# ooowedyn/InkLayer

Hardware: AMD Instinct MI355X
Metric: sketches/sec end-to-end (GroundingDINO+SAM) at 1024x1024 (higher is better)
Workload: dtype f16 (MFMA, f32 accumulate; f32 residual/norm/softmax; split-f16 = fp32-grade operands for patch-embed, neck, mask decoder); 1 GPU; full GroundingDINO Swin-T + SAM ViT-H pipeline, batch=8 per GPU, 1024x1024 synthetic sketches, 16 boxes/sketch, random-init weights; global_batch=8, parallelism=image-parallel x1

## Files before the change

inklayer_amd/build.py:

```python
from __future__ import annotations

import os
import subprocess
import sys
from concurrent.futures import ThreadPoolExecutor
from pathlib import Path

ROOT = Path(__file__).resolve().parent
CSRC = ROOT / "csrc"
LIBDIR = ROOT / "lib"
OBJDIR = LIBDIR / "obj"
LIB = LIBDIR / "libinklayer_hip.so"
HIPCC = os.environ.get("HIPCC", "/opt/rocm/bin/hipcc")
FLAGS = ["--offload-arch=gfx950", "-O3", "-std=c++17", "-fPIC", "-ffp-contract=off",
         "-mllvm", "-amdgpu-mfma-vgpr-form",

         "-Wall", "-Wno-unused-function", "-Wno-unused-variable"]


def _newest_header() -> float:
    hs = list(CSRC.glob("*.h")) + list((ROOT.parent / "include").glob("*.h"))
    return max(h.stat().st_mtime for h in hs)


NO_SPILL = {"ffn_fused.hip", "proj_ln.hip", "amg.hip", "layers.hip", "inpaint_ops.hip", "visualize.hip", "evaluate.hip",
            "gemm.hip", "attention_swin.hip", "biattn_wide.hip", "text_bert.hip"}


def _check_no_spill(src: Path, remarks: str) -> None:
    name = None
    for line in remarks.splitlines():
        if "Function Name:" in line:
            name = line.split("Function Name:")[1].split("[")[0].strip()
        elif "ScratchSize [bytes/lane]:" in line:
            n = int(line.split("ScratchSize [bytes/lane]:")[1].split("[")[0])
            if n != 0:
                raise RuntimeError(f"{src.name}: kernel {name} spills ({n} bytes of scratch per lane) - the kernels of "
                                   f"this file must stay in registers (see NO_SPILL); reduce register pressure")


def _compile(src: Path, force: bool, hdr_time: float) -> Path:
    obj = OBJDIR / (src.stem + ".o")
    if (not force and obj.exists() and obj.stat().st_mtime > src.stat().st_mtime
            and obj.stat().st_mtime > hdr_time):
        return obj
    guard = src.name in NO_SPILL
    cmd = [HIPCC, *FLAGS, *(["-Rpass-analysis=kernel-resource-usage", "-fno-caret-diagnostics"] if guard else []), "-c", str(src), "-o", str(obj)]
    r = subprocess.run(cmd, capture_output=True, text=True)
    if r.returncode != 0:
        raise RuntimeError(f"hipcc failed for {src.name}:\n{r.stdout}\n{r.stderr}")
    err = r.stderr
    if guard:
        try:
            _check_no_spill(src, err)
        except RuntimeError:
            obj.unlink(missing_ok=True)
            raise
        err = "\n".join(l for l in err.splitlines()
                        if "kernel-resource-usage" not in l and not l.startswith("In file included from"))
    if err.strip():
        sys.stderr.write(err)
    return obj


def build(force: bool = False, verbose: bool = True) -> Path:
    OBJDIR.mkdir(parents=True, exist_ok=True)
    srcs = sorted(CSRC.glob("*.hip"))
    if not srcs:
        raise RuntimeError("no HIP sources found")
    hdr_time = _newest_header()
    with ThreadPoolExecutor(max_workers=min(8, len(srcs))) as ex:
        objs = list(ex.map(lambda s: _compile(s, force, hdr_time), srcs))
    if (force or not LIB.exists()
            or any(o.stat().st_mtime > LIB.stat().st_mtime for o in objs)):
        cmd = [HIPCC, "--offload-arch=gfx950", "-shared", "-fPIC", "-o", str(LIB),
               *map(str, objs)]
        r = subprocess.run(cmd, capture_output=True, text=True)
        if r.returncode != 0:
            raise RuntimeError(f"link failed:\n{r.stdout}\n{r.stderr}")
    if verbose:
        print(f"[inklayer_amd.build] {LIB} ({LIB.stat().st_size >> 10} KiB, {len(srcs)} sources)")
    return LIB


if __name__ == "__main__":
    build(force="--force" in sys.argv)
```

inklayer_amd/csrc/attention_glob.hip:

```cpp
#include "mfma_util.h"
#include "../../include/inklayer_hip.h"

namespace {

typedef int i32x4 __attribute__((ext_vector_type(4)));

constexpr int HD = 80, NT = 256, NQK = 5, NB = 3, CH = 10;
constexpr int KROW = 176, VROW = 192;
constexpr int TILE = 64 * KROW + 64 * VROW;
constexpr int RWROW = 272;
constexpr int LDS_BYTES = 2 * TILE + 256 * RWROW;
constexpr int OROW = 176;
static_assert(4 * 64 * OROW <= 2 * TILE, "the output tiles fit the K/V buffers");
constexpr float NEG = -1e30f;
constexpr float THR = 12.0f;

struct Sub {
  f16x8 qf[NQK];
  f32x16 s0, s1;
  uint32_t pw[16];
  f32x16 o[NB];
  float m, nm;
  float mx, mx2, ea, eb, fa, fb;
  __device__ __forceinline__ f16x8 pfrag(int ks) const {
    typedef uint32_t u32x4 __attribute__((ext_vector_type(4)));
    return __builtin_bit_cast(f16x8, (u32x4){pw[4 * ks], pw[4 * ks + 1], pw[4 * ks + 2], pw[4 * ks + 3]});
  }
};

__device__ __forceinline__ void s_mfma(int j, const f16x8 (&kfa)[NQK], const f16x8 (&kfb)[NQK], Sub& u) {
  const int s = j >> 1;
  if (j & 1) u.s1 = mfma32(kfb[s], u.qf[s], u.s1);
  else u.s0 = mfma32(kfa[s], u.qf[s], u.s0);
}
__device__ __forceinline__ void pv_mfma(int j, const f16x8 (&vf)[12], Sub& u) {
  u.o[j % 3] = mfma32(vf[j], u.pfrag(j / 3), u.o[j % 3]);
}
__device__ __forceinline__ void sm_max(int g, Sub& u) {
  if (g == 0) {
    u.mx = max3_at(u.s0[0], u.s0[1], u.s0[2]);
    u.mx2 = max3_at(u.s0[3], u.s0[4], u.s0[5]);
    u.mx = max3_at(u.mx, u.s0[6], u.s0[7]);
    u.mx2 = max3_at(u.mx2, u.s0[8], u.s0[9]);
    u.mx = max3_at(u.mx, u.s0[10], u.s0[11]);
    u.mx2 = max3_at(u.mx2, u.s0[12], u.s0[13]);
  } else if (g == 1) {
    u.mx = max3_at(u.mx, u.s0[14], u.s0[15]);
    u.mx2 = max3_at(u.mx2, u.s1[0], u.s1[1]);
    u.mx = max3_at(u.mx, u.s1[2], u.s1[3]);
    u.mx2 = max3_at(u.mx2, u.s1[4], u.s1[5]);
    u.mx = max3_at(u.mx, u.s1[6], u.s1[7]);
  } else {
    u.mx2 = max3_at(u.mx2, u.s1[8], u.s1[9]);
    u.mx = max3_at(u.mx, u.s1[10], u.s1[11]);
    u.mx2 = max3_at(u.mx2, u.s1[12], u.s1[13]);
    u.mx = max3_at(u.mx, u.s1[14], u.s1[15]);
    u.mx = fmaxf(u.mx, u.mx2);
  }
}
template <bool FIRST>
__device__ __forceinline__ void sm_decide(Sub& u, float c, float rh) {
  float x = u.mx, y = u.mx;
  asm volatile("s_nop 1\n\tv_permlane32_swap_b32 %0, %1" : "+v"(x), "+v"(y));
  const float mc = (fmaxf(x, y) + rh) * c;
  if constexpr (FIRST) {
    u.m = mc;
  } else {
    if (__any(mc - u.m > THR)) {
      const float m_new = fmaxf(u.m, mc);
      const float alpha = __builtin_amdgcn_exp2f(u.m - m_new);
#pragma unroll
      for (int i = 0; i < NB; ++i)
#pragma unroll
        for (int r2 = 0; r2 < 16; ++r2) u.o[i][r2] *= alpha;
      u.m = m_new;
    }
  }
  u.nm = rh * c - u.m;
}
__device__ __forceinline__ void sm_exp(int i, Sub& u, float c) {
  float pa = 0.f, pb = 0.f;
  if (i >= 2 && i < 18) { pa = u.ea; pb = u.eb; }
  if (i >= 1 && i < 17) {
    u.ea = exp2_at(u.fa);
    u.eb = exp2_at(u.fb);
  }
  if (i < 16) {
    float a, b;
    if (i < 8) { a = u.s0[2 * i]; b = u.s0[2 * i + 1]; }
    else { a = u.s1[2 * i - 16]; b = u.s1[2 * i - 15]; }
    u.fa = fma_at(a, c, u.nm);
    u.fb = fma_at(b, c, u.nm);
  }
  if (i >= 2 && i < 18) u.pw[i - 2] = cvt_pk_at(pa, pb);
}
template <bool FIRST>
__device__ __forceinline__ void sm_first(int g, Sub& u, float c, float rh) {
  if (g < 3) sm_max(g, u);
  else if (g == 3) sm_decide<FIRST>(u, c, rh);
  else sm_exp(g - 4, u, c);
}
__device__ __forceinline__ void sm_second(int g, Sub& u, float c) { sm_exp(8 + g, u, c); }

template <bool RF16>
__global__ __launch_bounds__(NT) __attribute__((amdgpu_waves_per_eu(1, 1))) void glob4_attn_kernel(InkAttn p) {
  using RT = std::conditional_t<RF16, f16, float>;
  extern __shared__ __attribute__((aligned(16))) char smem[];
  asm volatile("v_accvgpr_write_b32 a255, %0" ::"v"(0) : "a255");
  char* sRW = smem + 2 * TILE;

  const int tid = threadIdx.x, lane = tid & 63;
  const int wave = __builtin_amdgcn_readfirstlane(tid >> 6);
  const int lq = lane & 31, hh = lane >> 5;
  const int nqb = p.n_q >> 8;
  const int blk = xcd_remap((int)blockIdx.x, (int)gridDim.x);
  const int bh = blk / nqb, qb = blk - bh * nqb;
  const int b = bh / p.n_heads, h = bh - b * p.n_heads;
  const int ntiles = p.n_k >> 6;
  const int64_t qrow0 = p.q_batch_rows ? (int64_t)p.q_batch_rows[b] : (int64_t)b * p.n_q;
  const int64_t kvb = p.kv_batch_rows ? (int64_t)p.kv_batch_rows[b] : (int64_t)b * p.n_k;
  const int qlA = wave * 32 + lq, qlB = 128 + wave * 32 + lq;

  Sub A, B;
  auto load_q = [&](Sub& u, int ql) {
    const int64_t q = (int64_t)qb * 256 + ql;
    const f16* Qrow = (const f16*)p.Q + (qrow0 + q) * p.ldq + h * HD + 8 * hh;
#pragma unroll
    for (int s = 0; s < NQK; ++s) u.qf[s] = *(const f16x8*)(Qrow + 16 * s);
  };
  load_q(A, qlA);
  load_q(B, qlB);
  {
    const RT* RW = (const RT*)p.rel_w + ((int64_t)bh * p.n_q + (int64_t)qb * 256) * 64;
#pragma unroll
    for (int it = 0; it < 16; ++it) {
      const int ci = it * NT + tid, q = ci >> 4, c4 = ci & 15;
      if constexpr (RF16) {
        const f16x4 v = *(const f16x4*)(RW + q * 64 + c4 * 4);
        *(f32x4*)(sRW + q * RWROW + c4 * 16) = (f32x4){(float)v[0], (float)v[1], (float)v[2], (float)v[3]};
      } else {
        *(f32x4*)(sRW + q * RWROW + c4 * 16) = *(const f32x4*)(RW + q * 64 + c4 * 4);
      }
    }
  }
  const RT* RHA = (const RT*)p.rel_h + ((int64_t)bh * p.n_q + (int64_t)qb * 256 + qlA) * 64;
  const RT* RHB = (const RT*)p.rel_h + ((int64_t)bh * p.n_q + (int64_t)qb * 256 + qlB) * 64;
  for (int i = tid; i < 2 * 64 * 2; i += NT) {
    const int buf = i >> 7, row = (i >> 1) & 63, pc = i & 1;
    f16x8 z = {0, 0, 0, 0, 0, 0, 0, 0};
    if (pc == 0) { z[0] = (f16)1; z[4] = (f16)1; }
    *(f16x8*)(smem + buf * TILE + 64 * KROW + row * VROW + (CH + pc) * 16) = z;
  }

  const char* Kg = (const char*)p.K + (kvb * p.ldk + h * HD) * 2;
  const char* Vg = (const char*)p.V + (kvb * p.ldv + h * HD) * 2;
  uint32_t goff[5];
  int loff[5];
  bool isv[5];
#pragma unroll
  for (int it = 0; it < 5; ++it) {
    const int ci = it * NT + tid;
    const bool v = ci >= 640;
    const int cj = v ? ci - 640 : ci, row = cj / CH, cc = cj - row * CH;
    isv[it] = v;
    goff[it] = (uint32_t)(row * (v ? p.ldv : p.ldk) * 2 + cc * 16);
    loff[it] = v ? 64 * KROW + row * VROW + cc * 16 : row * KROW + cc * 16;
  }
  f16x8 stg[2][5];
  const char* gp[5];
#pragma unroll
  for (int it = 0; it < 5; ++it) gp[it] = (isv[it] ? Vg : Kg) + goff[it];
  const int64_t kstride = (int64_t)64 * p.ldk * 2, vstride = (int64_t)64 * p.ldv * 2;
  auto g_load = [&](int tile, auto SET, auto IT) {
    constexpr int set = decltype(SET)::value, it = decltype(IT)::value;
    stg[set][it] = *(const f16x8*)gp[it];
    const int64_t step = tile + 1 < ntiles ? (isv[it] ? vstride : kstride) : 0;
    gp[it] += step;
  };
  auto l_write = [&](int buf, auto SET, auto IT) {
    constexpr int set = decltype(SET)::value, it = decltype(IT)::value;
    *(f16x8*)(smem + buf * TILE + loff[it]) = stg[set][it];
  };
  static_for<0, 5>([&](auto it) { g_load(0, ic<0>{}, it); });
  static_for<0, 5>([&](auto it) { g_load(1, ic<1>{}, it); });
  static_for<0, 5>([&](auto it) { l_write(0, ic<0>{}, it); });
  static_for<0, 5>([&](auto it) { l_write(1, ic<1>{}, it); });
  static_for<0, 5>([&](auto it) { g_load(2, ic<0>{}, it); });
  __syncthreads();

  const float c = p.scale * 1.44269504088896340736f;
  const int koff0 = lq * KROW + hh * 16;
  const int koff1 = (32 + lq) * KROW + hh * 16;
  const int voff = 64 * KROW + (4 * hh + ((lane & 15) >> 2)) * VROW + (16 * ((lane >> 4) & 1) + 4 * (lane & 3)) * 2;
#pragma unroll
  for (int i = 0; i < NB; ++i)
#pragma unroll
    for (int r = 0; r < 16; ++r) A.o[i][r] = B.o[i][r] = 0.f;
  A.m = B.m = NEG;
  A.nm = B.nm = 0.f;
  f16x8 kfa[NQK], kfb[NQK], vf[12];
  auto read_k = [&](int buf, int s) {
    kfa[s] = *(const f16x8*)(smem + buf * TILE + koff0 + s * 32);
    kfb[s] = *(const f16x8*)(smem + buf * TILE + koff1 + s * 32);
  };
  auto read_v = [&](int buf, int j) {
    const char* base = smem + buf * TILE + voff + (16 * (j / 3)) * VROW + (j % 3) * 64;
    const f16x4 a0 = tr_read(base);
    const f16x4 a1 = tr_read(base + 8 * VROW);
    vf[j] = (f16x8){a0[0], a0[1], a0[2], a0[3], a1[0], a1[1], a1[2], a1[3]};
  };
#define GAP() __builtin_amdgcn_sched_barrier(0)

  auto read_rw = [&](Sub& u, int ql, int g) {
    const f32x4 a = *(const f32x4*)(sRW + ql * RWROW + (8 * g + 4 * hh) * 4);
    const f32x4 c2 = *(const f32x4*)(sRW + ql * RWROW + (32 + 8 * g + 4 * hh) * 4);
#pragma unroll
    for (int r = 0; r < 4; ++r) { u.s0[4 * g + r] = a[r]; u.s1[4 * g + r] = c2[r]; }
  };
  float rhA = (float)RHA[0], rhB = (float)RHB[0];
#pragma unroll
  for (int g = 0; g < 4; ++g) { read_rw(A, qlA, g); read_rw(B, qlB, g); }
#pragma unroll
  for (int s = 0; s < NQK; ++s) read_k(0, s);
#pragma unroll
  for (int j = 0; j < 10; ++j) s_mfma(j, kfa, kfb, A);
  GAP();

  auto tile_iter = [&](int t, auto PAR_, auto FIRST_) {
    constexpr int PAR = decltype(PAR_)::value;
    constexpr bool FIRST = decltype(FIRST_)::value;
    float rhA1 = 0.f, rhB1 = 0.f;
    if constexpr (FIRST) {
      static_for<0, 10>([&](auto g_) {
        constexpr int g = decltype(g_)::value;
        s_mfma(g, kfa, kfb, B);
        sm_first<true>(g, A, c, rhA);
        read_v(PAR, g);
        if constexpr (g == 9) { read_v(PAR, 10); read_v(PAR, 11); }
        if constexpr (g % 4 == 1) g_load(t + 3, ic<1 - PAR>{}, ic<g / 4>{});
        GAP();
      });
      static_for<10, 12>([&](auto g_) { sm_first<true>(decltype(g_)::value, A, c, rhA); GAP(); });
      static_for<0, 10>([&](auto g_) {
        constexpr int g = decltype(g_)::value;
        sm_second(g, A, c);
        if constexpr (g == 2) g_load(t + 3, ic<1 - PAR>{}, ic<3>{});
        if constexpr (g == 6) g_load(t + 3, ic<1 - PAR>{}, ic<4>{});
        GAP();
      });
    } else {
      static_for<0, 12>([&](auto g_) {
        constexpr int g = decltype(g_)::value;
        pv_mfma(g, vf, B);
        sm_first<false>(g, A, c, rhA);
        if constexpr (g % 4 == 2) g_load(t + 3, ic<1 - PAR>{}, ic<g / 4>{});
        if constexpr (g >= 8) read_rw(B, qlB, g - 8);
        GAP();
      });
      static_for<0, 10>([&](auto g_) {
        constexpr int g = decltype(g_)::value;
        s_mfma(g, kfa, kfb, B);
        sm_second(g, A, c);
        read_v(PAR, g);
        if constexpr (g == 9) { read_v(PAR, 10); read_v(PAR, 11); }
        if constexpr (g == 3) g_load(t + 3, ic<1 - PAR>{}, ic<3>{});
        if constexpr (g == 7) g_load(t + 3, ic<1 - PAR>{}, ic<4>{});
        GAP();
      });
    }
    asm volatile("s_waitcnt lgkmcnt(0)" ::: "memory");
    __builtin_amdgcn_s_barrier();
    asm volatile("" ::: "memory");
    static_for<0, 12>([&](auto g_) {
      constexpr int g = decltype(g_)::value;
      pv_mfma(g, vf, A);
      sm_first<FIRST>(g, B, c, rhB);
      if constexpr (g < NQK) read_k(1 - PAR, g);
      if constexpr (g == 5) { rhA1 = (float)RHA[(t + 1) & 63]; rhB1 = (float)RHB[(t + 1) & 63]; }
      if constexpr (g >= 6 && g % 2 == 0) l_write(PAR, ic<PAR>{}, ic<(g - 6) / 2>{});
      if constexpr (g >= 8) read_rw(A, qlA, g - 8);
      GAP();
    });
    static_for<0, 10>([&](auto g_) {
      constexpr int g = decltype(g_)::value;
      s_mfma(g, kfa, kfb, A);
      sm_second(g, B, c);
      if constexpr (g == 2) l_write(PAR, ic<PAR>{}, ic<3>{});
      if constexpr (g == 6) l_write(PAR, ic<PAR>{}, ic<4>{});
      GAP();
    });
    rhA = rhA1;
    rhB = rhB1;
  };

  tile_iter(0, ic<0>{}, std::true_type{});
  tile_iter(1, ic<1>{}, std::false_type{});
  for (int t = 2; t < ntiles; t += 2) {
    tile_iter(t, ic<0>{}, std::false_type{});
    tile_iter(t + 1, ic<1>{}, std::false_type{});
  }
  static_for<0, 12>([&](auto g_) { pv_mfma(decltype(g_)::value, vf, B); });
#undef GAP

  __syncthreads();
  char* myO = smem + wave * 64 * OROW;
  auto stage_o = [&](const Sub& u, int row0) {
    const float inv = 1.0f / u.o[2][8];
    char* dst = myO + (row0 + lq) * OROW + 8 * hh;
#pragma unroll
    for (int i = 0; i < NB; ++i)
#pragma unroll
      for (int g = 0; g < 4; ++g) {
        if (32 * i + 8 * g < HD) {
          const f16x4 v = {(f16)(u.o[i][4 * g] * inv), (f16)(u.o[i][4 * g + 1] * inv),
                           (f16)(u.o[i][4 * g + 2] * inv), (f16)(u.o[i][4 * g + 3] * inv)};
          *(f16x4*)(dst + (32 * i + 8 * g) * 2) = v;
        }
      }
  };
  stage_o(A, 0);
  stage_o(B, 32);
  f16* Ob = (f16*)p.O + ((int64_t)b * p.n_q + (int64_t)qb * 256) * p.ldo + h * HD;
#pragma unroll
  for (int j = 0; j < 10; ++j) {
    const int idx = j * 64 + lane, row = idx / CH, ch = idx - row * CH;
    const f16x8 v = *(const f16x8*)(myO + row * OROW + ch * 16);
    const int ql = row < 32 ? wave * 32 + row : 128 + wave * 32 + row - 32;
    *(f16x8*)(Ob + (int64_t)ql * p.ldo + ch * 8) = v;
  }
}

}

__attribute__((visibility("hidden"))) int ink_glob4_attn_launch(const InkAttn& p, hipStream_t s) {
  ink_dyn_lds<glob4_attn_kernel<false>>(LDS_BYTES);
  ink_dyn_lds<glob4_attn_kernel<true>>(LDS_BYTES);
  const int grid = p.n_batch * p.n_heads * (p.n_q >> 8);
  if (p.rel_f16) {
    hipLaunchKernelGGL(glob4_attn_kernel<true>, dim3(grid), dim3(NT), LDS_BYTES, s, p);
  } else {
    hipLaunchKernelGGL(glob4_attn_kernel<false>, dim3(grid), dim3(NT), LDS_BYTES, s, p);
  }
  return ink_launch_status();
}
```

Baseline: 118.4 sketches/s.

## Reschedule global attention inner loop with AGPR-operand QK MFMAs and finer LDS interleave

```diff
diff --git a/inklayer_amd/build.py b/inklayer_amd/build.py
--- a/inklayer_amd/build.py
+++ b/inklayer_amd/build.py
@@ -24,7 +24,7 @@
 
 
 NO_SPILL = {"ffn_fused.hip", "proj_ln.hip", "amg.hip", "layers.hip", "inpaint_ops.hip", "visualize.hip", "evaluate.hip",
-            "gemm.hip", "attention_swin.hip", "biattn_wide.hip", "text_bert.hip"}
+            "gemm.hip", "attention_swin.hip", "biattn_wide.hip", "text_bert.hip", "attention_glob.hip"}
 
 
 def _check_no_spill(src: Path, remarks: str) -> None:
diff --git a/inklayer_amd/csrc/attention_glob.hip b/inklayer_amd/csrc/attention_glob.hip
--- a/inklayer_amd/csrc/attention_glob.hip
+++ b/inklayer_amd/csrc/attention_glob.hip
@@ -28,10 +28,13 @@
   }
 };
 
+__device__ __forceinline__ void mfma32_aa(const f16x8& a, const f16x8& b, f32x16& c) {
+  asm("v_mfma_f32_32x32x16_f16 %0, %1, %2, %0" : "+v"(c) : "a"(a), "a"(b));
+}
 __device__ __forceinline__ void s_mfma(int j, const f16x8 (&kfa)[NQK], const f16x8 (&kfb)[NQK], Sub& u) {
   const int s = j >> 1;
-  if (j & 1) u.s1 = mfma32(kfb[s], u.qf[s], u.s1);
-  else u.s0 = mfma32(kfa[s], u.qf[s], u.s0);
+  if (j & 1) mfma32_aa(kfb[s], u.qf[s], u.s1);
+  else mfma32_aa(kfa[s], u.qf[s], u.s0);
 }
 __device__ __forceinline__ void pv_mfma(int j, const f16x8 (&vf)[12], Sub& u) {
   u.o[j % 3] = mfma32(vf[j], u.pfrag(j / 3), u.o[j % 3]);
@@ -66,7 +69,7 @@
   if constexpr (FIRST) {
     u.m = mc;
   } else {
-    if (__any(mc - u.m > THR)) {
+    if (__builtin_expect(__any(mc - u.m > THR), 0)) {
       const float m_new = fmaxf(u.m, mc);
       const float alpha = __builtin_amdgcn_exp2f(u.m - m_new);
 #pragma unroll
@@ -143,6 +146,7 @@
       }
     }
   }
+  using RB = std::conditional_t<RF16, uint16_t, uint32_t>;
   const RT* RHA = (const RT*)p.rel_h + ((int64_t)bh * p.n_q + (int64_t)qb * 256 + qlA) * 64;
   const RT* RHB = (const RT*)p.rel_h + ((int64_t)bh * p.n_q + (int64_t)qb * 256 + qlB) * 64;
   for (int i = tid; i < 2 * 64 * 2; i += NT) {
@@ -217,7 +221,25 @@
 #pragma unroll
     for (int r = 0; r < 4; ++r) { u.s0[4 * g + r] = a[r]; u.s1[4 * g + r] = c2[r]; }
   };
-  float rhA = (float)RHA[0], rhB = (float)RHB[0];
+  auto rh_fetch = [&](const RT* base, int t) { return (uint32_t) * (const RB*)(base + (t & 63)); };
+  auto rh_value = [&](uint32_t bits) {
+    if constexpr (RF16) return (float)__builtin_bit_cast(f16, (uint16_t)bits);
+    else return __builtin_bit_cast(float, bits);
+  };
+  auto read_rw1 = [&](Sub& u, int ql, int i) {
+    const int g = i & 3;
+    const f32x4 a = *(const f32x4*)(sRW + ql * RWROW + (32 * (i >> 2) + 8 * g + 4 * hh) * 4);
+#pragma unroll
+    for (int r = 0; r < 4; ++r) {
+      if (i < 4) u.s0[4 * g + r] = a[r]; else u.s1[4 * g + r] = a[r];
+    }
+  };
+  auto read_k1 = [&](int buf, int i) {
+    const int s = i >> 1;
+    if (i & 1) kfb[s] = *(const f16x8*)(smem + buf * TILE + koff1 + s * 32);
+    else kfa[s] = *(const f16x8*)(smem + buf * TILE + koff0 + s * 32);
+  };
+  float rhA = rh_value(rh_fetch(RHA, 0)), rhB = rh_value(rh_fetch(RHB, 0));
 #pragma unroll
   for (int g = 0; g < 4; ++g) { read_rw(A, qlA, g); read_rw(B, qlB, g); }
 #pragma unroll
@@ -229,11 +251,12 @@
   auto tile_iter = [&](int t, auto PAR_, auto FIRST_) {
     constexpr int PAR = decltype(PAR_)::value;
     constexpr bool FIRST = decltype(FIRST_)::value;
-    float rhA1 = 0.f, rhB1 = 0.f;
+    uint32_t rhA1 = 0, rhB1 = 0;
     if constexpr (FIRST) {
       static_for<0, 10>([&](auto g_) {
         constexpr int g = decltype(g_)::value;
         s_mfma(g, kfa, kfb, B);
+        GAP();
         sm_first<true>(g, A, c, rhA);
         read_v(PAR, g);
         if constexpr (g == 9) { read_v(PAR, 10); read_v(PAR, 11); }
@@ -244,6 +267,7 @@
       static_for<0, 10>([&](auto g_) {
         constexpr int g = decltype(g_)::value;
         sm_second(g, A, c);
+        if constexpr (g < 4) read_rw1(A, qlA, g); else if constexpr (g >= 8) read_rw1(A, qlA, g - 4);
         if constexpr (g == 2) g_load(t + 3, ic<1 - PAR>{}, ic<3>{});
         if constexpr (g == 6) g_load(t + 3, ic<1 - PAR>{}, ic<4>{});
         GAP();
@@ -252,17 +276,20 @@
       static_for<0, 12>([&](auto g_) {
         constexpr int g = decltype(g_)::value;
         pv_mfma(g, vf, B);
+        GAP();
         sm_first<false>(g, A, c, rhA);
         if constexpr (g % 4 == 2) g_load(t + 3, ic<1 - PAR>{}, ic<g / 4>{});
-        if constexpr (g >= 8) read_rw(B, qlB, g - 8);
+        if constexpr (g < 2) read_rw1(B, qlB, 6 + g);
+        if constexpr (g >= 1) read_v(PAR, g - 1);
         GAP();
       });
       static_for<0, 10>([&](auto g_) {
         constexpr int g = decltype(g_)::value;
         s_mfma(g, kfa, kfb, B);
+        GAP();
         sm_second(g, A, c);
-        read_v(PAR, g);
-        if constexpr (g == 9) { read_v(PAR, 10); read_v(PAR, 11); }
+        if constexpr (g < 4) read_rw1(A, qlA, g); else if constexpr (g >= 8) read_rw1(A, qlA, g - 4);
+        if constexpr (g == 0) read_v(PAR, 11);
         if constexpr (g == 3) g_load(t + 3, ic<1 - PAR>{}, ic<3>{});
         if constexpr (g == 7) g_load(t + 3, ic<1 - PAR>{}, ic<4>{});
         GAP();
@@ -274,23 +301,26 @@
     static_for<0, 12>([&](auto g_) {
       constexpr int g = decltype(g_)::value;
       pv_mfma(g, vf, A);
+      GAP();
       sm_first<FIRST>(g, B, c, rhB);
-      if constexpr (g < NQK) read_k(1 - PAR, g);
-      if constexpr (g == 5) { rhA1 = (float)RHA[(t + 1) & 63]; rhB1 = (float)RHB[(t + 1) & 63]; }
-      if constexpr (g >= 6 && g % 2 == 0) l_write(PAR, ic<PAR>{}, ic<(g - 6) / 2>{});
-      if constexpr (g >= 8) read_rw(A, qlA, g - 8);
+      if constexpr (g < 10) read_k1(1 - PAR, g);
+      if constexpr (g == 10) { rhA1 = rh_fetch(RHA, t + 1); rhB1 = rh_fetch(RHB, t + 1); }
+      if constexpr (g < 2) read_rw1(A, qlA, 6 + g);
       GAP();
     });
     static_for<0, 10>([&](auto g_) {
       constexpr int g = decltype(g_)::value;
       s_mfma(g, kfa, kfb, A);
+      GAP();
       sm_second(g, B, c);
-      if constexpr (g == 2) l_write(PAR, ic<PAR>{}, ic<3>{});
-      if constexpr (g == 6) l_write(PAR, ic<PAR>{}, ic<4>{});
+      if constexpr (g < 4) read_rw1(B, qlB, g); else if constexpr (g >= 8) read_rw1(B, qlB, g - 4);
+      if constexpr (g == 1 || g == 3) l_write(PAR, ic<PAR>{}, ic<g / 2>{});
+      if constexpr (g >= 5 && g <= 7) l_write(PAR, ic<PAR>{}, ic<g - 3>{});
       GAP();
     });
-    rhA = rhA1;
-    rhB = rhB1;
+    asm volatile("" : "+v"(rhA1), "+v"(rhB1));
+    rhA = rh_value(rhA1);
+    rhB = rh_value(rhB1);
   };
 
   tile_iter(0, ic<0>{}, std::true_type{});
```

New measurement: 119.3 sketches/s (median of 5 runs). Within noise of the previous version (+0.7%).
